# akopich/spark-gp

Measured on AMD Instinct MI355X. Metric: rows/sec (full GP fit: BCM hyperopt + PPA), higher is better.
Workload: dtype fp32; 1 GPU; model=ARD-RBF GP regression, m=1000, expert=100, maxIter=100, restart=False, rows=10000000, dim=32, active_set=1000, expert_size=100, ppa_precision=mixed, parallelism=expert-parallel dp1

## Files before the change

spark_gp_amd/ops/csrc/linalg_lds.h:

```cpp
#pragma once
#include <hip/hip_runtime.h>
#include <math.h>

#ifndef WG
#define WG 512
#endif
#define NB 32

typedef __attribute__((ext_vector_type(4))) float mfma_f32x4_t;

__device__ inline double wave_sum(double v) {
#pragma unroll
  for (int off = 32; off; off >>= 1) v += __shfl_down(v, off, 64);
  return v;
}

__device__ inline double block_sum(double v, double* red, int tid) {
  v = wave_sum(v);
  if ((tid & 63) == 0) red[tid >> 6] = v;
  __syncthreads();
  if (tid == 0) {
    double s = 0;
#pragma unroll
    for (int w = 0; w < WG / 64; ++w) s += red[w];
    red[0] = s;
  }
  __syncthreads();
  double out = red[0];
  __syncthreads();
  return out;
}

__device__ inline float bcast_lane(float x, int src) {
  return __builtin_bit_cast(
      float, __builtin_amdgcn_readlane(__builtin_bit_cast(int, x), src));
}

__device__ inline void tri_decode(int f, int& a, int& b) {
  a = (int)((sqrtf(8.f * (float)f + 1.f) - 1.f) * 0.5f);
  while ((a + 1) * (a + 2) / 2 <= f) ++a;
  while (a * (a + 1) / 2 > f) --a;
  b = f - a * (a + 1) / 2;
}

__device__ inline float dotv(const float* p, const float* q, int c0,
                             int c1) {
  float s = 0.f;
  int c = c0;
  for (; c < c1 && (c & 3); ++c) s += p[c] * q[c];
  float4 a4 = {0.f, 0.f, 0.f, 0.f};
  for (; c + 3 < c1; c += 4) {
    const float4 a = *(const float4*)(p + c);
    const float4 b = *(const float4*)(q + c);
    a4.x += a.x * b.x;
    a4.y += a.y * b.y;
    a4.z += a.z * b.z;
    a4.w += a.w * b.w;
  }
  s += (a4.x + a4.y) + (a4.z + a4.w);
  for (; c < c1; ++c) s += p[c] * q[c];
  return s;
}

__device__ inline float dot8_unfused(const float* p, const float* q) {
#pragma clang fp contract(off)
  const float4 a0 = *(const float4*)p, b0 = *(const float4*)q;
  const float4 a1 = *(const float4*)(p + 4), b1 = *(const float4*)(q + 4);
  const float m0 = a0.x * b0.x, m1 = a0.y * b0.y;
  const float m2 = a0.z * b0.z, m3 = a0.w * b0.w;
  const float n0 = a1.x * b1.x, n1 = a1.y * b1.y;
  const float n2 = a1.z * b1.z, n3 = a1.w * b1.w;
  const float x = (0.f + m0) + n0, y = (0.f + m1) + n1;
  const float z = (0.f + m2) + n2, w = (0.f + m3) + n3;
  return 0.f + ((x + y) + (z + w));
}

__device__ inline float dotm(const float* p, const float* q, int sq,
                             int c0, int c1) {
  float s = 0.f;
  int c = c0;
  for (; c < c1 && (c & 3); ++c) s += p[c] * q[c * sq];
  float s0 = 0.f, s1 = 0.f, s2 = 0.f, s3 = 0.f;
  for (; c + 3 < c1; c += 4) {
    const float4 a = *(const float4*)(p + c);
    s0 += a.x * q[c * sq];
    s1 += a.y * q[(c + 1) * sq];
    s2 += a.z * q[(c + 2) * sq];
    s3 += a.w * q[(c + 3) * sq];
  }
  s += (s0 + s1) + (s2 + s3);
  for (; c < c1; ++c) s += p[c] * q[c * sq];
  return s;
}

__device__ inline float dot4(const float* p, int sp, const float* q, int sq,
                             int c0, int c1) {
  float s0 = 0.f, s1 = 0.f, s2 = 0.f, s3 = 0.f;
  int c = c0;
  for (; c + 3 < c1; c += 4) {
    s0 += p[c * sp] * q[c * sq];
    s1 += p[(c + 1) * sp] * q[(c + 1) * sq];
    s2 += p[(c + 2) * sp] * q[(c + 2) * sq];
    s3 += p[(c + 3) * sp] * q[(c + 3) * sq];
  }
  for (; c < c1; ++c) s0 += p[c * sp] * q[c * sq];
  return (s0 + s1) + (s2 + s3);
}

__device__ inline void wave_lds_sync() {
  __builtin_amdgcn_fence(__ATOMIC_RELEASE, "wavefront");
  asm volatile("s_waitcnt lgkmcnt(0)" ::: "memory");
  __builtin_amdgcn_wave_barrier();
  __builtin_amdgcn_fence(__ATOMIC_ACQUIRE, "wavefront");
}

__device__ inline void chol_invert_lower(float* Abuf, float* Tbuf,
                                         const int k, const int SA,
                                         const int tid_in, int* bad,
                                         double* misc,
                                         unsigned long long* jclk = nullptr) {
  int tid = tid_in;
  const int nblk = (k + NB - 1) / NB;
  for (int J = 0; J < nblk; ++J) {
    asm volatile("" : "+v"(tid));
    const int lane = tid & 63;
    const int jb = J * NB;
    const int bs = min(NB, k - jb);
    float* D = Abuf + (size_t)jb * SA + jb;
    const int pj = jb - NB;
    unsigned long long jt0 = 0, jt1 = 0;
    if (jclk && tid == 0) jt0 = wall_clock64();

    if (J > 0) {
      for (int f = tid; f < bs * bs; f += WG) {
        const int r = f / bs, c = f - r * bs;
        if (c > r) continue;
        const int i = jb + r, cc = jb + c;
        Abuf[(size_t)i * SA + cc] -=
            dotv(Abuf + (size_t)i * SA + pj,
                 Abuf + (size_t)cc * SA + pj, 0, NB);
      }
      __syncthreads();
    }
    if (jclk && (tid == 0 || tid == 64)) jt1 = wall_clock64();

    const int nq = (bs + 7) / 8;
    float* Vq = Tbuf;
    float* TS = Tbuf + 256;
    const int t0r = jb + bs;
    const int nrp = k - t0r;
    const int ntri_rest = nrp * (nrp + 1) / 2;
    if (tid < 64) {
      __builtin_amdgcn_s_setprio(1);
      int w0ok = 1;
      for (int q = 0; q < nq; ++q) {
        const int qb = q * 8;
        const int sbs = min(8, bs - qb);
        {
          const int j = lane & 7;
          float row[8];
#pragma unroll
          for (int c = 0; c < 8; ++c)
            row[c] = (j < sbs && c < sbs && c <= j)
                         ? D[(size_t)(qb + j) * SA + qb + c]
                         : (c == j ? 1.f : 0.f);
          bool ok = true, nonfin = false;
          float mprod = 1.f;
          int expsum = 0;
          float myrs = 1.f;
          float rsv = 1.f;
#pragma unroll
          for (int ss = 0; ss < 8; ++ss) {
            float l[8];
#pragma unroll
            for (int c = 0; c < 8; ++c) l[c] = bcast_lane(row[ss], c);
            const float piv = l[ss];
            if (ss < sbs) {
              const bool fin = isfinite(piv);
              nonfin = nonfin || (ok && !fin);
              ok = ok && fin && (piv > 0.f);
              mprod *= __builtin_amdgcn_frexp_mantf(piv);
              expsum += __builtin_amdgcn_frexp_expf(piv);
            }
            const float rs = rsqrtf(piv);
            if (j == ss) myrs = rs;
            const float w = (j > ss) ? rs * row[ss] : 0.f;
#pragma unroll
            for (int c = ss + 1; c < 8; ++c) row[c] -= (rs * l[c]) * w;
          }
#pragma unroll
          for (int c = 0; c < 8; ++c) {
            rsv = bcast_lane(myrs, c);
            row[c] *= rsv;
          }
          if (lane < 8 && j < sbs) {
#pragma unroll
            for (int c = 0; c < 8; ++c)
              if (c <= j) D[(size_t)(qb + j) * SA + qb + c] = row[c];
          }
          float v[8];
#pragma unroll
          for (int i = 0; i < 8; ++i) v[i] = (i == j) ? myrs : 0.f;
#pragma unroll
          for (int i = 0; i < 8; ++i) {
            float rowi[8];
#pragma unroll
            for (int c = 0; c < 8; ++c) rowi[c] = bcast_lane(row[c], i);
            if (j < i) {
              float sacc = 0.f;
#pragma unroll
              for (int c = 0; c < 8; ++c)
                if (c >= j && c < i) sacc += rowi[c] * v[c];
              v[i] = -sacc * __builtin_amdgcn_rcpf(rowi[i]);
            }
          }
          if (lane < 8) {
#pragma unroll
            for (int i = 0; i < 8; ++i) Vq[q * 64 + i * 8 + j] = v[i];
          }
          w0ok = __builtin_amdgcn_readlane((int)ok, 0);
          if (lane == 0) {
            if (!ok) {
              if (*bad == 0) *bad = nonfin ? 2 : 1;
            } else {
              misc[0] += (double)__logf(mprod)
                         + (double)expsum * 0.6931471805599453;
            }
          }
        }
        if (!w0ok) break;
        wave_lds_sync();
        const int p0 = qb + sbs;
        const int pr = bs - p0;
        if (pr > 0) {
          if (lane < pr) {
            float* ap = D + (size_t)(p0 + lane) * SA + qb;
            const float4 a0 = *(const float4*)ap;
            const float4 a1 = *(const float4*)(ap + 4);
            const float ar[8] = {a0.x, a0.y, a0.z, a0.w,
                                 a1.x, a1.y, a1.z, a1.w};
            const float* vr = Vq + q * 64;
            float o[8];
#pragma unroll
            for (int c = 0; c < 8; ++c) {
              float sacc = 0.f;
#pragma unroll
              for (int t = 0; t <= c; ++t)
                sacc = __builtin_fmaf(ar[t], vr[c * 8 + t], sacc);
              o[c] = sacc;
            }
            *(float4*)ap = make_float4(o[0], o[1], o[2], o[3]);
            *(float4*)(ap + 4) = make_float4(o[4], o[5], o[6], o[7]);
          }
          wave_lds_sync();
          const int wd = pr + 1, tot = ((pr + 1) >> 1) * wd;
          const float rwd = 1.f / (float)wd;
          for (int f0 = lane; f0 < tot; f0 += 128) {
            float* tp[2];
            const float *pa[2], *pb[2];
            bool on[2];
#pragma unroll
            for (int u = 0; u < 2; ++u) {
              const int f = f0 + 64 * u;
              const int r = (int)(((float)f + 0.5f) * rwd);
              const int c = f - r * wd;
              const bool lo = c <= r;
              on[u] = f < tot && (lo || pr - 1 - r != r);
              const int a = on[u] ? (lo ? r : pr - 1 - r) : 0;
              const int b = on[u] ? (lo ? c : c - r - 1) : 0;
              tp[u] = D + (size_t)(p0 + a) * SA + p0 + b;
              pa[u] = D + (size_t)(p0 + a) * SA + qb;
              pb[u] = D + (size_t)(p0 + b) * SA + qb;
            }
            const float s0 = dot8_unfused(pa[0], pb[0]);
            const float s1 = dot8_unfused(pa[1], pb[1]);
            if (on[0]) *tp[0] -= s0;
            if (on[1]) *tp[1] -= s1;
          }
          wave_lds_sync();
        }
      }
      __builtin_amdgcn_s_setprio(0);
      if (jclk && tid == 0) jclk[2] += wall_clock64() - jt1;
    } else if (J > 0) {
      for (int f = tid - 64; f < nrp * bs; f += WG - 64) {
        const int r = f / bs, c = f - r * bs;
        const int i = t0r + r, cc = jb + c;
        Abuf[(size_t)i * SA + cc] -=
            dotv(Abuf + (size_t)i * SA + pj,
                 Abuf + (size_t)cc * SA + pj, 0, NB);
      }
      for (int f = tid - 64; f < ntri_rest; f += WG - 64) {
        int a, b;
        tri_decode(f, a, b);
        const int i = t0r + a, c = t0r + b;
        Abuf[(size_t)i * SA + c] -=
            dotv(Abuf + (size_t)i * SA + pj,
                 Abuf + (size_t)c * SA + pj, 0, NB);
      }
      if (jclk && tid == 64) jclk[3] += wall_clock64() - jt1;
    }
    __syncthreads();
    if (*bad == 0) {
      for (int Jq = nq - 1; Jq >= 0; --Jq) {
        const int jb8 = Jq * 8;
        const int nblks = nq - 1 - Jq;
        for (int f = tid; f < nblks * 64; f += WG) {
          const int blk = f >> 6;
          const int ib = (Jq + 1 + blk) * 8;
          const int i = (f >> 3) & 7, j = f & 7;
          const int gi = ib + i;
          float u = 0.f;
          if (gi < bs && jb8 + j < bs) {
            u = dotm(D + (size_t)gi * SA, D + jb8 + j, SA,
                     jb8 + 8, min(gi + 1, bs));
          }
          TS[f] = u;
        }
        __syncthreads();
        for (int f = tid; f < nblks * 64; f += WG) {
          const int blk = f >> 6;
          const int ib = (Jq + 1 + blk) * 8;
          const int i = (f >> 3) & 7, j = f & 7;
          const int gi = ib + i;
          if (gi >= bs || jb8 + j >= bs) continue;
          float sacc = 0.f;
          const float* ts = TS + blk * 64 + i * 8;
          const float* vv = Vq + Jq * 64;
#pragma unroll
          for (int t = 0; t < 8; ++t) sacc += ts[t] * vv[t * 8 + j];
          D[(size_t)gi * SA + jb8 + j] = -sacc;
        }
        for (int f = tid; f < 64; f += WG) {
          const int i = (f >> 3) & 7, j = f & 7;
          const int gi = jb8 + i, gj = jb8 + j;
          if (gi < bs && gj <= gi) D[(size_t)gi * SA + gj] = Vq[Jq * 64 + f];
        }
        __syncthreads();
      }
    }
    if (jclk && tid == 0) {
      const unsigned long long t2 = wall_clock64();
      jclk[0] += jt1 - jt0;
      jclk[1] += t2 - jt1;
      jt0 = t2;
    }
    if (*bad) break;

    const int t0 = jb + bs;
    const int nr = k - t0;
    if (nr > 0) {
      for (int f = tid; f < nr * bs; f += WG) {
        int r = f / bs, c = f - r * bs;
        Tbuf[r * 36 + c] = Abuf[(size_t)(t0 + r) * SA + jb + c];
      }
      __syncthreads();
      {
        const int w8 = tid >> 6;
        const int fl16 = lane & 15, fkg = lane >> 4;
        const int nti = (nr + 15) / 16, ntj = (bs + 15) / 16;
        for (int t = w8; t < nti * ntj; t += WG / 64) {
          const int ti = t / ntj, tj = t - ti * ntj;
          mfma_f32x4_t a = {0.f, 0.f, 0.f, 0.f};
          const int fr = ti * 16 + fl16;
          const int fc = tj * 16 + fl16;
          for (int c0 = 0; c0 < bs; c0 += 4) {
            const int tt = c0 + fkg;
            const float av = (fr < nr && tt < bs)
                                 ? Tbuf[fr * 36 + tt] : 0.f;
            const float bv = (fc < bs && tt <= fc)
                                 ? D[(size_t)fc * SA + tt] : 0.f;
            a = __builtin_amdgcn_mfma_f32_16x16x4f32(av, bv, a, 0, 0, 0);
          }
#pragma unroll
          for (int r = 0; r < 4; ++r) {
            const int gr = ti * 16 + fkg * 4 + r;
            const int gc = tj * 16 + fl16;
            if (gr < nr && gc < bs)
              Abuf[(size_t)(t0 + gr) * SA + jb + gc] = a[r];
          }
        }
      }
      __syncthreads();
    }
    if (jclk && tid == 0) jclk[4] += wall_clock64() - jt0;
  }

  if (*bad) return;
  unsigned long long dt0 = 0;
  if (jclk && tid == 0) dt0 = wall_clock64();
  for (int J = nblk - 2; J >= 0; --J) {
    asm volatile("" : "+v"(tid));
    const int lane = tid & 63;
    const int jb = J * NB;
    const int bs = NB;
    const int t0 = jb + bs;
    const int nr = k - t0;
    const int w8 = tid >> 6;
    const int fl16 = lane & 15, fkg = lane >> 4;
    const int nti = (nr + 15) / 16, ntj = (bs + 15) / 16;
    for (int t = w8; t < nti * ntj; t += WG / 64) {
      const int ti = t / ntj, tj = t - ti * ntj;
      mfma_f32x4_t a = {0.f, 0.f, 0.f, 0.f};
      const int fr = t0 + ti * 16 + fl16;
      const int fj = tj * 16 + fl16;
      for (int c0 = t0; c0 < k; c0 += 4) {
        const int cc = c0 + fkg;
        const float av = (fr < k && cc < k && cc <= fr)
                             ? Abuf[(size_t)fr * SA + cc] : 0.f;
        const float bv = (cc < k && fj < bs)
                             ? Abuf[(size_t)cc * SA + jb + fj] : 0.f;
        a = __builtin_amdgcn_mfma_f32_16x16x4f32(av, bv, a, 0, 0, 0);
      }
#pragma unroll
      for (int r = 0; r < 4; ++r) {
        const int gr = ti * 16 + fkg * 4 + r;
        const int gc = tj * 16 + fl16;
        if (gr < nr && gc < bs) Tbuf[gr * 36 + gc] = a[r];
      }
    }
    __syncthreads();
    for (int t = w8; t < nti * ntj; t += WG / 64) {
      const int ti = t / ntj, tj = t - ti * ntj;
      mfma_f32x4_t a = {0.f, 0.f, 0.f, 0.f};
      const int fr = ti * 16 + fl16;
      const int fj = tj * 16 + fl16;
      for (int c0 = 0; c0 < bs; c0 += 4) {
        const int tt = c0 + fkg;
        const float av = (fr < nr && tt < bs)
                             ? Tbuf[fr * 36 + tt] : 0.f;
        const float bv = (tt < bs && fj < bs && tt >= fj)
                             ? Abuf[(size_t)(jb + tt) * SA + jb + fj]
                             : 0.f;
        a = __builtin_amdgcn_mfma_f32_16x16x4f32(av, bv, a, 0, 0, 0);
      }
#pragma unroll
      for (int r = 0; r < 4; ++r) {
        const int gr = ti * 16 + fkg * 4 + r;
        const int gc = tj * 16 + fl16;
        if (gr < nr && gc < bs)
          Abuf[(size_t)(t0 + gr) * SA + jb + gc] = -a[r];
      }
    }
    __syncthreads();
  }
  if (jclk && tid == 0) jclk[5] += wall_clock64() - dt0;
}
```

Measured before the change: 25.17 million rows/s.

## Assemble 32x32 diagonal-block inverse with MFMA in one wave

Replaces the block-wide back-substitution loop that built the inverse of the 32x32 diagonal Cholesky block (several __syncthreads rounds over all 512 threads) with a single-wave routine that combines the 8x8 sub-inverses using 16x16x4 fp32 MFMA ops. The 8x8 factorisation now computes the inverse alongside elimination, using FMA-based updates in place of a separate triangular solve, and writes it with vectorised float4 stores. This removes block barriers and scalar dot products from the critical path. It adds heavy index and predicate logic that assumes a block size of 32, and it changes the rounding order.

After: 26.84 million rows/s, median of 6. +6.6%, better.

```diff
diff --git a/spark_gp_amd/ops/csrc/linalg_lds.h b/spark_gp_amd/ops/csrc/linalg_lds.h
--- a/spark_gp_amd/ops/csrc/linalg_lds.h
+++ b/spark_gp_amd/ops/csrc/linalg_lds.h
@@ -112,6 +112,86 @@
   asm volatile("s_waitcnt lgkmcnt(0)" ::: "memory");
   __builtin_amdgcn_wave_barrier();
   __builtin_amdgcn_fence(__ATOMIC_ACQUIRE, "wavefront");
+}
+
+__device__ inline void assemble_diag_inverse(float* D, const int SA,
+                                             const float* Vq, const int bs,
+                                             const int nq, const int lane) {
+  const int fl = lane & 15, kg = lane >> 4;
+  const int fp = fl >> 3, f7 = fl & 7;
+  float dg[4];
+#pragma unroll
+  for (int u = 0; u < 4; ++u) dg[u] = Vq[lane + 64 * u];
+  float a1[4], b1[4], a2[4], a3[4], vd[4], a4[4];
+  const int lrow = 16 * fp + 8 + f7;
+  const bool hrow = 16 + fl < bs;
+#pragma unroll
+  for (int s = 0; s < 4; ++s) {
+    const int kk = 4 * kg + s, k7 = kk & 7, kp = kk >> 3;
+    const bool c1 = kp == fp && lrow < bs;
+    const bool c2 = kp == fp && 2 * fp < nq;
+    const bool c3 = kp != fp && 2 * kp + 1 < nq;
+    const bool c4 = kp == fp && 2 + fp < nq;
+    const float x1 = D[c1 ? (size_t)lrow * SA + 16 * fp + k7 : 0];
+    const float x2 = Vq[c2 ? (2 * fp) * 64 + k7 * 8 + f7 : 0];
+    const float x3 = Vq[c3 ? (2 * kp + 1) * 64 + f7 * 8 + k7 : 0];
+    const float x4 = D[hrow ? (size_t)(16 + fl) * SA + kk : 0];
+    const float x5 = Vq[c4 ? (2 + fp) * 64 + f7 * 8 + k7 : 0];
+    vd[s] = Vq[kp * 64 + k7 * 8 + f7];
+    a1[s] = c1 ? x1 : 0.f;
+    b1[s] = c2 ? x2 : 0.f;
+    a2[s] = c3 ? x3 : 0.f;
+    a3[s] = hrow ? x4 : 0.f;
+    a4[s] = c4 ? x5 : 0.f;
+  }
+#pragma unroll
+  for (int u = 0; u < 4; ++u) {
+    const int i = lane >> 3, j = lane & 7;
+    const int gi = u * 8 + i;
+    if (gi < bs && j <= i) D[(size_t)gi * SA + u * 8 + j] = dg[u];
+  }
+  if (nq < 2) return;
+  mfma_f32x4_t w = {0.f, 0.f, 0.f, 0.f};
+  mfma_f32x4_t r1 = {0.f, 0.f, 0.f, 0.f};
+#pragma unroll
+  for (int s = 0; s < 4; ++s)
+    w = __builtin_amdgcn_mfma_f32_16x16x4f32(a1[s], b1[s], w, 0, 0, 0);
+#pragma unroll
+  for (int s = 0; s < 4; ++s)
+    r1 = __builtin_amdgcn_mfma_f32_16x16x4f32(a2[s], w[s], r1, 0, 0, 0);
+#pragma unroll
+  for (int s = 0; s < 4; ++s) {
+    const int row = 4 * kg + s;
+    const int gr = 16 * fp + 8 + (row & 7);
+    if ((row >> 3) != fp && gr < bs)
+      D[(size_t)gr * SA + 16 * fp + f7] = -r1[s];
+  }
+  if (nq < 3) return;
+  mfma_f32x4_t w2 = {0.f, 0.f, 0.f, 0.f};
+#pragma unroll
+  for (int s = 0; s < 4; ++s) {
+    const int kp = (4 * kg + s) >> 3;
+    const float bv = (kp == fp) ? vd[s] : (kp > fp ? -r1[s] : 0.f);
+    w2 = __builtin_amdgcn_mfma_f32_16x16x4f32(a3[s], bv, w2, 0, 0, 0);
+  }
+  wave_lds_sync();
+  float a5[4];
+#pragma unroll
+  for (int s = 0; s < 4; ++s) {
+    const int kk = 4 * kg + s, k7 = kk & 7, kp = kk >> 3;
+    const bool c5 = fp > kp && 24 + f7 < bs;
+    const float x = D[c5 ? (size_t)(24 + f7) * SA + 16 + k7 : 0];
+    a5[s] = c5 ? x : a4[s];
+  }
+  mfma_f32x4_t r2 = {0.f, 0.f, 0.f, 0.f};
+#pragma unroll
+  for (int s = 0; s < 4; ++s)
+    r2 = __builtin_amdgcn_mfma_f32_16x16x4f32(a5[s], w2[s], r2, 0, 0, 0);
+#pragma unroll
+  for (int s = 0; s < 4; ++s) {
+    const int gr = 16 + 4 * kg + s;
+    if (gr < bs) D[(size_t)gr * SA + fl] = -r2[s];
+  }
 }
 
 __device__ inline void chol_invert_lower(float* Abuf, float* Tbuf,
@@ -146,7 +226,6 @@
 
     const int nq = (bs + 7) / 8;
     float* Vq = Tbuf;
-    float* TS = Tbuf + 256;
     const int t0r = jb + bs;
     const int nrp = k - t0r;
     const int ntri_rest = nrp * (nrp + 1) / 2;
@@ -159,21 +238,25 @@
         {
           const int j = lane & 7;
           float row[8];
-#pragma unroll
-          for (int c = 0; c < 8; ++c)
+          float inv[8];
+#pragma unroll
+          for (int c = 0; c < 8; ++c) {
             row[c] = (j < sbs && c < sbs && c <= j)
                          ? D[(size_t)(qb + j) * SA + qb + c]
                          : (c == j ? 1.f : 0.f);
+            inv[c] = (c == j) ? 1.f : 0.f;
+          }
           bool ok = true, nonfin = false;
           float mprod = 1.f;
           int expsum = 0;
           float myrs = 1.f;
-          float rsv = 1.f;
 #pragma unroll
           for (int ss = 0; ss < 8; ++ss) {
-            float l[8];
-#pragma unroll
-            for (int c = 0; c < 8; ++c) l[c] = bcast_lane(row[ss], c);
+            float l[8], pinv[8];
+#pragma unroll
+            for (int c = ss; c < 8; ++c) l[c] = bcast_lane(row[ss], c);
+#pragma unroll
+            for (int c = 0; c < ss; ++c) pinv[c] = bcast_lane(inv[c], ss);
             const float piv = l[ss];
             if (ss < sbs) {
               const bool fin = isfinite(piv);
@@ -184,39 +267,27 @@
             }
             const float rs = rsqrtf(piv);
             if (j == ss) myrs = rs;
-            const float w = (j > ss) ? rs * row[ss] : 0.f;
-#pragma unroll
-            for (int c = ss + 1; c < 8; ++c) row[c] -= (rs * l[c]) * w;
-          }
-#pragma unroll
-          for (int c = 0; c < 8; ++c) {
-            rsv = bcast_lane(myrs, c);
-            row[c] *= rsv;
-          }
-          if (lane < 8 && j < sbs) {
-#pragma unroll
-            for (int c = 0; c < 8; ++c)
-              if (c <= j) D[(size_t)(qb + j) * SA + qb + c] = row[c];
-          }
-          float v[8];
-#pragma unroll
-          for (int i = 0; i < 8; ++i) v[i] = (i == j) ? myrs : 0.f;
-#pragma unroll
-          for (int i = 0; i < 8; ++i) {
-            float rowi[8];
-#pragma unroll
-            for (int c = 0; c < 8; ++c) rowi[c] = bcast_lane(row[c], i);
-            if (j < i) {
-              float sacc = 0.f;
+            const float m = (j > ss) ? row[ss] * (rs * rs) : 0.f;
+#pragma unroll
+            for (int c = ss + 1; c < 8; ++c)
+              row[c] = __builtin_fmaf(-m, l[c], row[c]);
+#pragma unroll
+            for (int c = 0; c < ss; ++c)
+              inv[c] = __builtin_fmaf(-m, pinv[c], inv[c]);
+            if (j > ss) inv[ss] = -m;
+            row[ss] *= rs;
+          }
+#pragma unroll
+          for (int c = 0; c < 8; ++c) inv[c] *= myrs;
+          if (lane < 8) {
+            if (j < sbs) {
 #pragma unroll
               for (int c = 0; c < 8; ++c)
-                if (c >= j && c < i) sacc += rowi[c] * v[c];
-              v[i] = -sacc * __builtin_amdgcn_rcpf(rowi[i]);
+                if (c <= j) D[(size_t)(qb + j) * SA + qb + c] = row[c];
             }
-          }
-          if (lane < 8) {
-#pragma unroll
-            for (int i = 0; i < 8; ++i) Vq[q * 64 + i * 8 + j] = v[i];
+            float* vo = Vq + q * 64 + j * 8;
+            *(float4*)vo = make_float4(inv[0], inv[1], inv[2], inv[3]);
+            *(float4*)(vo + 4) = make_float4(inv[4], inv[5], inv[6], inv[7]);
           }
           w0ok = __builtin_amdgcn_readlane((int)ok, 0);
           if (lane == 0) {
@@ -280,8 +351,14 @@
           wave_lds_sync();
         }
       }
+      unsigned long long jt2 = 0;
+      if (jclk && tid == 0) {
+        jt2 = wall_clock64();
+        jclk[2] += jt2 - jt1;
+      }
+      if (w0ok) assemble_diag_inverse(D, SA, Vq, bs, nq, lane);
       __builtin_amdgcn_s_setprio(0);
-      if (jclk && tid == 0) jclk[2] += wall_clock64() - jt1;
+      if (jclk && tid == 0) jclk[6] += wall_clock64() - jt2;
     } else if (J > 0) {
       for (int f = tid - 64; f < nrp * bs; f += WG - 64) {
         const int r = f / bs, c = f - r * bs;
@@ -301,44 +378,6 @@
       if (jclk && tid == 64) jclk[3] += wall_clock64() - jt1;
     }
     __syncthreads();
-    if (*bad == 0) {
-      for (int Jq = nq - 1; Jq >= 0; --Jq) {
-        const int jb8 = Jq * 8;
-        const int nblks = nq - 1 - Jq;
-        for (int f = tid; f < nblks * 64; f += WG) {
-          const int blk = f >> 6;
-          const int ib = (Jq + 1 + blk) * 8;
-          const int i = (f >> 3) & 7, j = f & 7;
-          const int gi = ib + i;
-          float u = 0.f;
-          if (gi < bs && jb8 + j < bs) {
-            u = dotm(D + (size_t)gi * SA, D + jb8 + j, SA,
-                     jb8 + 8, min(gi + 1, bs));
-          }
-          TS[f] = u;
-        }
-        __syncthreads();
-        for (int f = tid; f < nblks * 64; f += WG) {
-          const int blk = f >> 6;
-          const int ib = (Jq + 1 + blk) * 8;
-          const int i = (f >> 3) & 7, j = f & 7;
-          const int gi = ib + i;
-          if (gi >= bs || jb8 + j >= bs) continue;
-          float sacc = 0.f;
-          const float* ts = TS + blk * 64 + i * 8;
-          const float* vv = Vq + Jq * 64;
-#pragma unroll
-          for (int t = 0; t < 8; ++t) sacc += ts[t] * vv[t * 8 + j];
-          D[(size_t)gi * SA + jb8 + j] = -sacc;
-        }
-        for (int f = tid; f < 64; f += WG) {
-          const int i = (f >> 3) & 7, j = f & 7;
-          const int gi = jb8 + i, gj = jb8 + j;
-          if (gi < bs && gj <= gi) D[(size_t)gi * SA + gj] = Vq[Jq * 64 + f];
-        }
-        __syncthreads();
-      }
-    }
     if (jclk && tid == 0) {
       const unsigned long long t2 = wall_clock64();
       jclk[0] += jt1 - jt0;
```
